# HIITMetagenomics/dsm-framework

Measured on AMD Instinct MI355X. Metric: enumerated substrings/sec (Emax=2.0), higher is better.
Workload: dtype u32

## Files before the change

### dsm-framework_amd/csrc/engine.hip

```cpp
#include <sched.h>

#include <algorithm>
#include <atomic>
#include <chrono>
#include <cmath>
#include <condition_variable>
#include <cstdlib>
#include <cstring>
#include <deque>
#include <map>
#include <functional>
#include <memory>
#include <mutex>
#include <sstream>
#include <thread>
#include <type_traits>

#include "common.h"
#include "scan.h"
#include "setorder.h"
#include "stream_parse.h"
#include "lfstep.h"
#include "entropy_tables.h"
#include "textemit.h"
// ... 833 lines not shown
        bitsv[i] = w < nw ? candbits[wc] : 0ull;
        basev[i] = wscan[wc];
    }
#pragma unroll
    for (int i = 0; i < NPT; ++i) {
        const u32 w = w0 + (u32)i * stride;
        const u64 bits = bitsv[i];
        if (!bits) continue;
        const u64 base = basev[i];
        const bool mine = (bits >> lane) & 1;
        const u32 v = w * 64 + lane;
        const u32 cnt = mine ? (a.d > 1 ? (u32)nT[v] : 1u) : 0u;
        const u32 k = (u32)(base & 0xFFFFFFFFu) + bits_below_lane(bits);
        u32 o = k;
        if (a.d > 1) o = (u32)(base >> 32) + (wave_inclusive_scan<u32>(cnt) - cnt);
        if (!mine) continue;
        cand_node[k] = v;
        cand_poff[k] = o;
        const u64 j = v;
        if (a.exact_order == 1) {
            const u64 ord = order[v];
            for (u32 q = 0; q < cnt; ++q) {
                u32 g = (u32)((ord >> (4 * q)) & 15);
                ids[o] = g; freqs[o] = (u64)x_freq<P>(x, g, j); ++o;
            }
        } else if (a.exact_order == 2) {
            const u16* ord = order16 + (size_t)v * a.d;
            for (u32 q = 0; q < cnt; ++q) {
                u32 g = ord[q];
                ids[o] = g; freqs[o] = (u64)x_freq<P>(x, g, j); ++o;
            }
        } else {
            for (u32 g = 0; g < a.d; ++g) {
                u64 f = (u64)x_freq<P>(x, g, j);
                if (f) { ids[o] = g; freqs[o] = f; ++o; }
            }
        }
    }
}

template <typename P>
__global__ void keep_kernel(u32 F, Xchg x, const uint2* __restrict__ sa, uint4* __restrict__ srec, u8* __restrict__ clen) {
    u32 v = blockIdx.x * blockDim.x + threadIdx.x;
    if (v >= F) return;
    const uint2 a = sa[v];
    const u64 f = (u64)x_freq<P>(x, 0, v);
    const u64 w = f | ((u64)(x_pl<P>(x, 0, v) >> 4) << 61);
    srec[v] = make_uint4(a.x, a.y, (u32)w, (u32)(w >> 32));
    clen[v] = (u8)((f < 128 ? 1u : 1u + (u32)((64 - __clzll((long long)f) + 7) >> 3)) + 2u);
}

template <typename T, typename OwnT>
__global__ __launch_bounds__(256) void up_kernel(u32 F, const OwnT* __restrict__ own, Kids kids, const T* __restrict__ child_agg,
                                                 T* __restrict__ agg) {
    const int lane = threadIdx.x & 63;
    const u32 nw = (F + 63) >> 6, stride = gridDim.x * 4;
    const u32 w0 = (u32)__builtin_amdgcn_readfirstlane((int)(xcd_block() * 4 + (threadIdx.x >> 6)));
    KidWave kw[NPT];
    T s[NPT];
#pragma unroll
    for (int i = 0; i < NPT; ++i) {
        const u32 w = w0 + (u32)i * stride, wc = w < nw ? w : 0u;
        const u32 v = wc * 64 + lane;
        s[i] = v < F ? (own ? (T)own[v] : (T)1) : (T)0;
        if (child_agg) kid_wave(kids, wc, kw[i]);
    }
    if (child_agg) {
        T g[NPT][4];
#pragma unroll
        for (int i = 0; i < NPT; ++i)
#pragma unroll
            for (int c = 0; c < 4; ++c) g[i][c] = child_agg[((kw[i].p[c] >> lane) & 1) ? kw[i].c[c] + bits_below_lane(kw[i].p[c]) : 0u];
#pragma unroll
        for (int i = 0; i < NPT; ++i)
#pragma unroll
            for (int c = 0; c < 4; ++c) s[i] += ((kw[i].p[c] >> lane) & 1) ? g[i][c] : (T)0;
    }
#pragma unroll
    for (int i = 0; i < NPT; ++i) {
        const u32 w = w0 + (u32)i * stride, v = w * 64 + lane;
        if (w < nw && v < F) agg[v] = s[i];
    }
}
template <typename T>
__global__ __launch_bounds__(256) void up_bits_kernel(u32 F, const u64* __restrict__ ownbits, Kids kids, const T* __restrict__ child_agg,
                                                      T* __restrict__ agg) {
    const int lane = threadIdx.x & 63;
    const u32 nw = (F + 63) >> 6, stride = gridDim.x * 4;
    const u32 w0 = (u32)__builtin_amdgcn_readfirstlane((int)(xcd_block() * 4 + (threadIdx.x >> 6)));
    KidWave kw[NPT];
    T s[NPT];
#pragma unroll
    for (int i = 0; i < NPT; ++i) {
        const u32 w = w0 + (u32)i * stride, wc = w < nw ? w : 0u;
        s[i] = ownbits ? (T)((ownbits[wc] >> lane) & 1) : (T)0;
        if (child_agg) kid_wave(kids, wc, kw[i]);
    }
    if (child_agg) {
        T g[NPT][4];
#pragma unroll
        for (int i = 0; i < NPT; ++i)
#pragma unroll
            for (int c = 0; c < 4; ++c) g[i][c] = child_agg[((kw[i].p[c] >> lane) & 1) ? kw[i].c[c] + bits_below_lane(kw[i].p[c]) : 0u];
#pragma unroll
        for (int i = 0; i < NPT; ++i)
#pragma unroll
            for (int c = 0; c < 4; ++c) s[i] += ((kw[i].p[c] >> lane) & 1) ? g[i][c] : (T)0;
    }
#pragma unroll
    for (int i = 0; i < NPT; ++i) {
        const u32 w = w0 + (u32)i * stride, v = w * 64 + lane;
        if (w < nw && v < F) agg[v] = s[i];
    }
}
template <typename T>
__global__ __launch_bounds__(256) void down_kernel(u32 F, const T* __restrict__ start, T lead, Kids kids,
                                                   const T* __restrict__ child_agg, T* __restrict__ child_start) {
    const int lane = threadIdx.x & 63;
    const u32 nw = (F + 63) >> 6, stride = gridDim.x * 4;
    const u32 w0 = (u32)__builtin_amdgcn_readfirstlane((int)(xcd_block() * 4 + (threadIdx.x >> 6)));
    KidWave kw[NPT];
    T s[NPT];
#pragma unroll
    for (int i = 0; i < NPT; ++i) {
        const u32 w = w0 + (u32)i * stride, wc = w < nw ? w : 0u;
        const u32 v = wc * 64 + lane;
        kid_wave(kids, wc, kw[i]);
        s[i] = start[v < F ? v : 0u] + lead;
    }
    T g[NPT][3];
#pragma unroll
    for (int i = 0; i < NPT; ++i)
#pragma unroll
        for (int c = 0; c < 3; ++c) {
            const bool need = ((kw[i].p[c] >> lane) & 1) && ((((kw[i].p[1] >> lane) & 1) << 1 | ((kw[i].p[2] >> lane) & 1) << 2 | ((kw[i].p[3] >> lane) & 1) << 3) >> (c + 1)) != 0;
            g[i][c] = child_agg[need ? kw[i].c[c] + bits_below_lane(kw[i].p[c]) : 0u];
        }
#pragma unroll
    for (int i = 0; i < NPT; ++i) {
        const u32 w = w0 + (u32)i * stride;
        if (w >= nw) continue;
        const u32 m = (u32)((kw[i].p[0] >> lane) & 1) | ((u32)((kw[i].p[1] >> lane) & 1) << 1) | ((u32)((kw[i].p[2] >> lane) & 1) << 2) |
                      ((u32)((kw[i].p[3] >> lane) & 1) << 3);
        T acc = s[i];
#pragma unroll
        for (int c = 0; c < 4; ++c) {
            if ((m >> c) & 1u) {
                child_start[kw[i].c[c] + bits_below_lane(kw[i].p[c])] = acc;
                if (c < 3 && (m >> (c + 1))) acc += g[i][c];
            }
        }
    }
}

struct RankSlot {
    u32 k, level;
    __device__ explicit operator u32() const { return level; }
};
__global__ void cand_rank_kernel(u32 ncand, const u32* __restrict__ cand_node, const u32* __restrict__ cand_poff, u32 npairs,
                                 const u32* __restrict__ start, const u32* __restrict__ sub, u32 level, RankSlot* __restrict__ slot,
                                 u32* __restrict__ npair, const uint4* __restrict__ crec) {
    u32 k = blockIdx.x * blockDim.x + threadIdx.x;
    if (k >= ncand) return;
    u32 v = crec ? crec[k].x : cand_node[k];
    u32 r = start[v] + sub[v] - 1;
    slot[r] = RankSlot{k, level};
    if (npair) npair[r] = crec ? 1u : (k + 1 < ncand ? cand_poff[k + 1] : npairs) - cand_poff[k];
}

struct LevelDev {
    const uint2* pw;
    const u32* cand_node;
    const u32* cand_poff;
    const uint4* crec;
    const u32* ids;
    const u64* freqs;
};

constexpr int EMIT_MAX_CHUNKS = 8;
struct ChunkBounds { u32 tb[EMIT_MAX_CHUNKS + 1]; int n; };
__global__ void chunk_bounds_kernel(ChunkBounds cbs, const u32* __restrict__ path_off, const u32* __restrict__ pair_off, u32* __restrict__ out) {
    const int c = threadIdx.x;
    if (c <= cbs.n) { out[2 * c] = path_off[cbs.tb[c]]; out[2 * c + 1] = pair_off ? pair_off[cbs.tb[c]] : cbs.tb[c]; }
}

constexpr u8 EV_DROP = 0, EV_KEEP = 1, EV_HOST = 2;
struct FillVerdict {
    u8* keep;
    double* ent;
    u32* rel_path;
    u32* rel_pair;
    u32* freq32;
    u32* counts;
    const double* terms;
    const double* logn;
    const u32* bounds;
    u32 chunk, d;
    double emin, emax;
};
__global__ __launch_bounds__(256) void tuple_fill_kernel(u32 nlev, const LevelDev* __restrict__ lv, const u32* __restrict__ path_off,
                                                         const u32* __restrict__ pair_off, const RankSlot* __restrict__ slot, char* __restrict__ paths,
                                                         u32* __restrict__ ids, u64* __restrict__ freqs, u32 rank_lo, u32 rank_hi, FillVerdict fv) {
    constexpr u32 LDS_LEVELS = 1024;
    __shared__ const uint2* s_pw[LDS_LEVELS];
    __shared__ u32 s_text[256];
    const u32 nl = nlev < LDS_LEVELS ? nlev : LDS_LEVELS;
    for (u32 q = threadIdx.x; q < nl; q += blockDim.x) s_pw[q] = lv[q].pw;
    {
        const u32 b = threadIdx.x;
        s_text[b] = ((0x54474341u >> (8 * (b & 3))) & 0xFFu) | (((0x54474341u >> (8 * ((b >> 2) & 3))) & 0xFFu) << 8) |
                    (((0x54474341u >> (8 * ((b >> 4) & 3))) & 0xFFu) << 16) | (((0x54474341u >> (8 * ((b >> 6) & 3))) & 0xFFu) << 24);
    }
    __syncthreads();
    const u32 r = rank_lo + blockIdx.x * blockDim.x + threadIdx.x;
    if (r >= rank_hi) return;
    const u32 p_first = path_off[r], p_end = path_off[r + 1];
    const u32 o_first = pair_off ? pair_off[r] : r, o_end = pair_off ? pair_off[r + 1] : r + 1;
    const u32 lvl = p_end - p_first;
    const u32 k = slot[r].k;
    const LevelDev L = lv[lvl];
    const bool one = L.crec != nullptr;
    const uint4 cr = one ? L.crec[k] : make_uint4(0u, 0u, 0u, 0u);
    const u32 b = one ? k : L.cand_poff[k];
    u64 sumN = fv.d;
    double sl = 0;
    bool beyond = false;
    for (u32 q = b, o = o_first; o < o_end; ++q, ++o) {
        const u64 fq = one ? (((u64)cr.w << 32) | cr.z) : L.freqs[q];
        if (ids) ids[o] = one ? 0u : L.ids[q];
        if (fv.freq32) fv.freq32[o] = (u32)fq; else freqs[o] = fq;
        sumN += fq;
        if (fv.keep && !beyond) {
            if (fq < TERM_TAB) sl += fv.terms[fq]; else beyond = true;
        }
    }
    if (fv.keep) {
        beyond = beyond || sumN >= LOGN_TAB;
        u8 verdict = EV_HOST;
        if (!beyond) {
            const double en = fv.logn[sumN] - sl / (double)sumN;
            if (fv.ent) fv.ent[r] = en;
            verdict = (fv.emax > 0 && (en < fv.emin || en > fv.emax)) ? EV_DROP : EV_KEEP;
        }
        const u32 pb0 = fv.bounds[2 * fv.chunk], qb0 = fv.bounds[2 * fv.chunk + 1];
        fv.keep[r] = verdict;
        fv.rel_path[r + fv.chunk] = p_first - pb0;
        if (fv.rel_pair) fv.rel_pair[r + fv.chunk] = o_first - qb0;
        if (r + 1 == rank_hi) {
// ... 151 lines not shown
    const u32 last = top_rank[v] + top_lf[v] - 1;
    const u64 val = rbase + cumk[last] + kop[last];
    rval[v] = val;
    atomicAdd(&chunk[last], 1u + varint_len(val));
}

constexpr u32 STREAM_LDS_LEVELS = 1024;
__global__ __launch_bounds__(256) void stream_chunk_kernel(u32 rank0, u32 nleaf, u32 nlev, const uint4* const* __restrict__ srec_tab, const u64* const* __restrict__ rval_tab,
                                                           const u64* __restrict__ leaf_id, const u64* __restrict__ chunk_off, const u32* __restrict__ kop,
                                                           u8* __restrict__ out) {
    __shared__ const uint4* s_rec[STREAM_LDS_LEVELS];
    const u32 nl = nlev < STREAM_LDS_LEVELS ? nlev : STREAM_LDS_LEVELS;
    for (u32 q = threadIdx.x; q < nl; q += blockDim.x) s_rec[q] = srec_tab[q];
    __syncthreads();
    const u32 r = rank0 + blockIdx.x * blockDim.x + threadIdx.x;
    if (r >= nleaf) return;
    const u64 id = leaf_id[r];
    u32 l = (u32)(id >> 32), v = (u32)id;
    const u32 ko = kop[r];
    u8* po = out + chunk_off[r] + 2ull * ko;
    u8* pc = po;
    bool inopen = true, inclose = true;
    while (l >= 1 && (inopen || inclose)) {
        const uint4 rec = (l < STREAM_LDS_LEVELS ? s_rec[l] : srec_tab[l])[v];
        if (inopen) {
            po -= 2;
            const unsigned short head = (unsigned short)('(' | ((0x54474341u >> (8 * (rec.y & 3u))) & 0xFFu) << 8);
            __builtin_memcpy(po, &head, 2);
            if (!(rec.y & SREC_FIRST)) inopen = false;
        }
        if (inclose) {
            const u64 fw = srec_word(rec);
            const u64 f = fw & SREC_FREQ_MASK;
            const u32 lc = (0x4E54474341300000ull >> (8 * ((u32)(fw >> 61) + 2))) & 0xFFu;
            if (l > 6 && f < (1ull << 32)) {
                u64 tok;
                u32 n;
                if (f < 128) { tok = f | 0x80; n = 1; }
                else { const u32 ln = (u32)((64 - __clzll((long long)f) + 7) >> 3); tok = (u64)ln | (f << 8); n = 1 + ln; }
                tok |= ((u64)lc | ((u64)')' << 8)) << (8 * n);
                n += 2;
                if (n & 4) { const u32 wv = (u32)tok; __builtin_memcpy(pc, &wv, 4); pc += 4; tok >>= 32; }
                if (n & 2) { const unsigned short wv = (unsigned short)tok; __builtin_memcpy(pc, &wv, 2); pc += 2; tok >>= 16; }
                if (n & 1) { *pc = (u8)tok; pc += 1; }
            } else {
                pc += put_varint(pc, f);
                if (l <= 6) { *pc++ = 'R'; pc += put_varint(pc, rval_tab[l][v]); }
                *pc++ = (u8)lc;
                *pc++ = ')';
            }
            if (!(rec.y & SREC_LAST)) inclose = false;
        }
        v = rec.x;
        --l;
    }
}

struct Arena {
    u8* base = nullptr;
    size_t cap = 0, off = 0;
    template <class T> T* get(size_t n) {
        size_t bytes = ((n ? n : 1) * sizeof(T) + 255) & ~(size_t)255;
        if (off + bytes > cap) return nullptr;
        T* p = reinterpret_cast<T*>(base + off);
        off += bytes;
        return p;
    }
};

struct LevelHost {
    u32 n = 0;
    u32* slot = nullptr;
    uint2* pw = nullptr;
    u64* kplane = nullptr;
    u32* kcum = nullptr;
    Kids kids() const { Kids k; k.plane = kplane; k.cum = kcum; return k; }
    u64* cand_bits = nullptr;
    u32 ncand = 0, npairs = 0;
    u32* cand_node = nullptr;
    u32* cand_poff = nullptr;
    uint4* crec = nullptr;
    u32* ids = nullptr;
    u64* freqs = nullptr;
    u32* sub = nullptr;
    uint4* srec = nullptr;
    u8* clen = nullptr;
    u32* lf = nullptr;
    u32* top_rank = nullptr;
    u32* top_lf = nullptr;
    u64* rval = nullptr;
};

static inline dim3 grid_for(u64 n, int t = 256) { return dim3((unsigned)((n + t - 1) / t)); }

#define ARENA_GET(var, T, n)                                                                        \
    do {                                                                                            \
        (var) = arena.get<T>(n);                                                                    \
        if (!(var)) return fail(DSM_E_CAPACITY, "device arena exhausted: use a longer prefix or a larger arena_bytes"); \
    } while (0)

static unsigned host_threads() {
    static unsigned n = 0;
    if (!n) {
        const char* e = getenv("DSM_HOST_THREADS");
        long v = e ? atol(e) : 0;
        if (v <= 0) {
            cpu_set_t cs;
            v = sched_getaffinity(0, sizeof cs, &cs) == 0 ? CPU_COUNT(&cs) : 1;
            if (v > 16) v = 16;
        }
        n = (unsigned)(v < 1 ? 1 : v);
    }
    return n;
}

struct RawBuf {
    void* p = nullptr;
    size_t cap = 0;
    void* ensure(size_t n) {
        if (n > cap) {
            free(p);
            cap = n + n / 4 + 4096;
            p = malloc(cap);
        }
        return p;
    }
    ~RawBuf() { free(p); }
};
struct PinBuf {
    void* p = nullptr;
    size_t cap = 0;
    int ensure(size_t n) {
        if (n <= cap) return 0;
        if (p) (void)hipHostFree(p);
        p = nullptr;
        cap = 0;
        size_t want = n + n / 4 + 4096;
        hipError_t e = hipHostMalloc(&p, want);
        if (e != hipSuccess) return fail(DSM_E_NOMEM, std::string("hipHostMalloc: ") + hipGetErrorString(e));
        cap = want;
        return 0;
    }
    ~PinBuf() { if (p) (void)hipHostFree(p); }
};
struct DevGrow {
    void* p = nullptr;
    size_t cap = 0;
    int ensure(size_t n) {
        if (n <= cap) return 0;
        if (p) (void)hipFree(p);
        p = nullptr;
        cap = 0;
        size_t want = n + n / 4 + 4096;
        hipError_t e = hipMalloc(&p, want);
        if (e != hipSuccess) return fail(DSM_E_NOMEM, std::string("hipMalloc: ") + hipGetErrorString(e));
        cap = want;
        return 0;
    }
    ~DevGrow() { if (p) (void)hipFree(p); }
};
struct EmitSet {
    DevGrow dev[11];
    bool one_pair = false, narrow = false;
    hipEvent_t ready = nullptr;
    static constexpr int MAX_CHUNKS = EMIT_MAX_CHUNKS;
    int nchunk = 1;
    u32 cb[MAX_CHUNKS + 1] = {0};
// ... 1248 lines not shown
            s.crec_cap = (u32)(room < (size_t)F ? room : (size_t)F);
        }
        const bool fold = s.crec_cap > 0;
        if (nbp > 1) {
            if (!merged) hipLaunchKernelGGL(lite_count_kernel, dim3((nbp + 63) / 64), dim3(256), 0, st, splane[0], (F + 63) >> 6, cntraw, nbp, 3u, fold ? 1u : 0u);
            exclusive_scan<u32, u32>(merged ? cnt4 : cntraw, cnt4, (size_t)(fold ? 5 : 4) * nbp, scan_tmp, d_totals, st);
        }
        const bool fused_filter = s.filtered && nbp > 1;
        if (fused_filter) {
            ao.fa = filter_args(F, depth, w.order_mode); ao.candbits = me.cand_bits; ao.wsum = cand_wsum;
            if (ao.single) ao.cand_copy = 1;
            else ao.filter_on = 1;
        }
        if (fold) { ao.crec = reinterpret_cast<uint4*>(carena.base + carena.off); ao.crec_cap = s.crec_cap; }
        if (nbp == 1) hipLaunchKernelGGL((advance_down_kernel<P>), dim3(1), dim3(256), 0, st, x, ao);
        else if (lean) hipLaunchKernelGGL((advance_single_kernel<P>), dim3((nbp + 3) / 4), dim3(256), 0, st, x, ao);
        else hipLaunchKernelGGL((advance_wave_kernel<P>), dim3(nbp), dim3(256), 0, st, x, ao);
        if (s.filtered) {
            if (int erc = emit_filter(me, F, depth, x, cur, w.order_mode, !fused_filter, fold)) return erc;
        }
        return 0;
    }

    int publish(Walk& w, Sweep& s) {
        const u32 F = w.F, nbp = (F + TILE - 1) / TILE;
        const int nxt = w.cur() ^ 1;
        PublishArgs pa;
        memset(&pa, 0, sizeof pa);
        pa.total = nbp == 1 ? d_pub_tot : d_totals;
        pa.cmax_base = s.x.base; pa.cmax_bpr = s.x.bpr; pa.cmax_world = (u32)world;
        if (s.filtered) pa.cand = d_totals64;
        if (s.crec_cap) {
            pa.total = cnt4 + (size_t)4 * nbp;
            pa.grand = d_totals;
            pa.cand = nullptr;
        }
        pa.clear = reinterpret_cast<u32*>(multi ? xsend : xrecv[nxt]);
        pa.packet = reinterpret_cast<uint4*>(h_totals + 304); pa.seq = ++pub_seq;
        pa.next = spec_mode ? d_dyn : nullptr;
        pa.bc_header = owner_mode ? reinterpret_cast<uint4*>(bc_buf) : nullptr;
        hipLaunchKernelGGL(publish_kernel, dim3(1), dim3(64), 0, st, pa);
        if (owner_mode) {
            const size_t bc_bytes = bcast_bytes(F);
            DSM_HIP(hipMemcpyAsync(bc_buf + 16, w.L[w.depth].kplane, bc_bytes - 16, hipMemcpyDeviceToDevice, st));
            w.owed.disarm();
            if (prm.bcast(prm.owner_ctx, owner, bc_buf, bc_bytes, (void*)st)) return fail(DSM_E_SINK, "bcast callback failed");
            stats.exchange_bytes_sent += bc_bytes * (u64)(world - 1);
        }
        if (spec_mode) { if (int rc = launch_lf(w, w.depth + 1, 0, w.w16, w.w9, s.slot, (u64)F * 4)) return rc; }
        u32 pk[4];
        if (int rc = wait_packet(pk)) return rc;
        s.Fn = decode_level(pk[1], &s.w16, &s.w9);
        s.spec_hit = spec_mode && s.Fn > 0 && s.Fn <= level_cap(s.w16) && s.w16 == w.w16 && s.w9 == w.w9;
        if (spec_mode && !s.spec_hit) --stats.expand_launches;
        h_totals[300] = pk[2]; h_totals[301] = pk[3];
        if (int rc = check_width(s.Fn, s.w16)) return rc;
        if (owner_mode) {
            if (!s.Fn) w.owed.arm(16);
            else w.owed.arm_next((size_t)level_bytes(s.Fn, s.w16, s.w9), xrecv[nxt], bcast_bytes(s.Fn));
        }
        return 0;
    }
    int wait_packet(u32 pk[4]) {
        volatile u32* fl = h_totals + 304;
        u32 spins = 0;
        while (*fl != pub_seq) {
            if ((++spins & 0xFFFFu) == 0 && hipStreamQuery(st) != hipErrorNotReady) {
                DSM_HIP(hipStreamSynchronize(st));
                if (*fl != pub_seq) return fail(DSM_E_HIP, "publish kernel did not report");
                break;
            }
            __builtin_ia32_pause();
        }
        std::atomic_thread_fence(std::memory_order_acquire);
        for (int q = 0; q < 4; ++q) pk[q] = fl[q];
        return 0;
    }

    int commit(Walk& w, const Sweep& s, LevelHost& child) {
        const u32 F = w.F, Fn = s.Fn;
        const int cur = w.cur(), nxt = cur ^ 1;
        arena.off = s.mark;
        child.n = Fn;
        if (!Fn) return 0;
        if (self_mode) child.slot = arena.get<u32>(Fn);
        if (!stream_mode) child.pw = arena.get<uint2>(Fn);
        if (int rc = alloc_kids(child)) return rc;
        if (s.spec_hit) {
            stats.expand_slots += Fn;
            stats.expand_column_bytes += (u64)Fn * col_bytes(s.w16, s.w9);
        } else {
            if (int rc = launch_lf(w, w.depth + 1, Fn, s.w16, s.w9, child.slot)) return rc;
        }
        const Kids kids = w.L[w.depth].kids();
        if (!(w.o.emit || w.o.capture)) {}
        else if (w.order_mode == 1)
            hipLaunchKernelGGL((order_kernel<P>), grid_for(F), dim3(256), 0, st, F, s.x, nT[cur], order[cur], kids, order[nxt]);
        else if (w.order_mode == 2 && d <= 64)
            hipLaunchKernelGGL((order_big_kernel<P, 64>), grid_for(F, 64), dim3(64), 0, st, F, s.x, nT[cur], order16[cur], kids, order16[nxt]);
        else if (w.order_mode == 2)
            hipLaunchKernelGGL((order_big_kernel<P, 273>), grid_for(F, 64), dim3(64), 0, st, F, s.x, nT[cur], order16[cur], kids, order16[nxt]);
        if (w.order_mode && w.o.seed && w.depth + 1 == w.o.seed->depth) {
            const std::vector<u16>& so = w.o.seed->ord[0];
            if (int rc = upload_order(nxt, so.data(), so.size())) return rc;
        }
        return 0;
    }

    int capture_level(Walk& w, u32 Fn, const u32* slot, const uint2* pw) {
        NodeOrder* cap = w.o.capture;
        if (!Fn || !cap || w.depth + 1 != cap->depth) return 0;
        const int nxt = w.cur() ^ 1;
        const bool client = owner_mode && !is_owner;
        std::vector<u32> hs(Fn);
        std::vector<u16> hn(Fn);
        if (slot) DSM_HIP(hipMemcpyAsync(hs.data(), slot, (size_t)Fn * sizeof(u32), hipMemcpyDeviceToHost, st));
        else if (stream_mode) {
            std::vector<uint2> hr(Fn);
            DSM_HIP(hipMemcpyAsync(hr.data(), sa[nxt], (size_t)Fn * sizeof(uint2), hipMemcpyDeviceToHost, st));
            DSM_HIP(hipStreamSynchronize(st));
            for (u32 v = 0; v < Fn; ++v) hs[v] = hr[v].y & 3u;
        } else {
            std::vector<uint2> hp(Fn);
            DSM_HIP(hipMemcpyAsync(hp.data(), pw, (size_t)Fn * sizeof(uint2), hipMemcpyDeviceToHost, st));
            DSM_HIP(hipStreamSynchronize(st));
            for (u32 v = 0; v < Fn; ++v) hs[v] = (hp[v].y >> (2 * (w.depth % PW_CHUNK))) & 3u;
        }
        if (!client) DSM_HIP(hipMemcpyAsync(hn.data(), nT[nxt], (size_t)Fn * sizeof(u16), hipMemcpyDeviceToHost, st));
        DSM_HIP(hipStreamSynchronize(st));
        const u32 order_mode = client ? 0u : w.order_mode;
        cap->sym.clear();
        cap->ord.clear();
        for (u32 v = 0; v < Fn; ++v) {
            cap->sym.push_back(hs[v] & 3);
            std::vector<u16> o(d == 1 || client ? 1 : hn[v]);
            if (order_mode == 1) {
                u64 ord = 0;
                DSM_HIP(hipMemcpy(&ord, order[nxt] + v, sizeof(u64), hipMemcpyDeviceToHost));
                for (u32 k = 0; k < hn[v]; ++k) o[k] = (u16)((ord >> (4 * k)) & 15);
            } else if (order_mode == 2) {
                DSM_HIP(hipMemcpy(o.data(), order16[nxt] + (size_t)v * d, (size_t)hn[v] * sizeof(u16), hipMemcpyDeviceToHost));
            }
            cap->ord.push_back(o);
        }
        return 0;
    }

    void count_level(const Walk& w) {
        if (w.trace) {
            if (owner_mode && !is_owner) fprintf(stderr, "dsm level prefix=%s depth=%u F=%u (client of rank %d)\n", w.prefix.c_str(), w.depth, w.F, owner);
            else fprintf(stderr, "dsm level prefix=%s depth=%u F=%u\n", w.prefix.c_str(), w.depth, w.F);
        }
        stats.union_nodes += w.depth >= 1 ? w.F : 0;
        if (w.F > stats.max_frontier) stats.max_frontier = w.F;
        ++stats.levels;
    }
    void step(Walk& w, u32 Fn, bool w16, bool w9) {
        w.F = Fn;
        ++w.depth;
        w.w16 = w16;
        w.w9 = w9;
    }

    int finish_prefix(Walk& w, dsm_tuple_sink tsink, dsm_byte_sink bsink, void* ctx) {
        const u32 nlev = (u32)w.L.size();
        if (stream_mode) {
// ... 50 lines not shown
            std::vector<u64> sh((size_t)COUNTER_SHARDS * 8);
            DSM_HIP(hipMemcpy(sh.data(), d_counters, sh.size() * sizeof(u64), hipMemcpyDeviceToHost));
            for (int k = 0; k < COUNTER_SHARDS; ++k)
                for (int c = 0; c < NCOUNTERS; ++c) hc[c] += sh[(size_t)k * 8 + c];
#ifdef DSM_CLOCK_PROBE
            if (sh[7]) {
                double dur = 0, ramp = 0, tail = 0, meanbusy = 0;
                int nl = 0;
                const double W = (double)lfgeo.blocks * lfgeo.waves_per_block;
                for (int k = 1; k + 2 < COUNTER_SHARDS; k += 3) {
                    const u64 s0 = ~sh[(size_t)k * 8 + 6], s9 = sh[(size_t)k * 8 + 7], e0 = ~sh[(size_t)(k + 1) * 8 + 6], e9 = sh[(size_t)(k + 1) * 8 + 7];
                    if (!s9 || e9 - s0 < 5000) continue;
                    const double ms = (double)sh[(size_t)(k + 2) * 8 + 6] / W, me = (double)sh[(size_t)(k + 2) * 8 + 7] / W;
                    dur += (double)(e9 - s0); ramp += (double)(s9 - s0); tail += (double)(e9 - e0); meanbusy += me - ms; ++nl;
                }
                fprintf(stderr, "clock probe: %.1f MHz; %d launches >= 50 us: duration %.2f ms, first-to-last wave start %.2f ms, first-to-last wave end %.2f ms, mean wave busy %.2f ms\n",
                        (double)sh[6] / (double)sh[7] * 100.0, nl, dur * 1e-5, ramp * 1e-5, tail * 1e-5, meanbusy * 1e-5);
            }
#endif
        }
        stats.reported += hc[0];
        stats.lf_steps += hc[1];
        stats.rank_ops += hc[2];
        stats.index_lines += hc[3];
        stats.record_bytes += hc[4];
        stats.records_read += hc[5];
        return 0;
    }

    FilterArgs filter_args(u32 F, u32 depth, u32 order_mode) const {
        FilterArgs fa;
        fa.F = F; fa.depth = depth; fa.d = d; fa.pmin = prm.pmin; fa.pmax = prm.pmax; fa.mindepth = prm.mindepth;
        fa.emin = prm.emin; fa.emax = prm.emax; fa.exact_order = order_mode;
        return fa;
    }
    int emit_alloc(LevelHost& me, u32 F) {
        EARENA_GET(me.cand_bits, u64, ((size_t)F + 63) / 64);
        return 0;
    }
    int emit_filter(LevelHost& me, u32 F, u32 depth, const Xchg& xp, int cur, u32 order_mode, bool run_kernel, bool stored = false) {
        const FilterArgs fa = filter_args(F, depth, order_mode);
        if (run_kernel)
            hipLaunchKernelGGL((filter_kernel<P>), grid_npt(F), dim3(256), 0, st, fa, xp, nT[cur], me.kids(), samechild, me.cand_bits, cand_wsum);
        if (!stored) exclusive_scan<u64, u64>(cand_wsum, cand_wscan, ((size_t)F + 63) / 64, scan_tmp64, d_totals64, st);
        return 0;
    }
    int emit_store(LevelHost& me, u32 F, u32 depth, const Xchg& xp, int cur, u32 order_mode, u32 stored_cap = 0) {
        const FilterArgs fa = filter_args(F, depth, order_mode);
        u64 tot = 0;
        memcpy(&tot, h_totals + 300, sizeof tot);
        me.ncand = (u32)(tot & 0xFFFFFFFFu);
        me.npairs = (u32)(tot >> 32);
        if (stored_cap && me.ncand <= stored_cap) {
            if (me.ncand) {
                me.crec = carena.get<uint4>(me.ncand);
                if (!me.crec) return fail(DSM_E_HIP, "candidate arena: the block that held the records cannot be claimed");
            }
            stats.candidates += me.ncand;
            return 0;
        }
        if (stored_cap)
            exclusive_scan<u64, u64>(cand_wsum, cand_wscan, ((size_t)F + 63) / 64, scan_tmp64, d_totals64, st);
        if (me.ncand) {
            u32 nc = me.ncand;
            me.ncand = 0;
            EARENA_GET(me.cand_node, u32, nc);
            EARENA_GET(me.cand_poff, u32, nc);
            EARENA_GET(me.ids, u32, me.npairs);
            EARENA_GET(me.freqs, u64, me.npairs);
            me.ncand = nc;
            hipLaunchKernelGGL((cand_store_kernel<P>), grid_npt(F), dim3(256), 0, st, fa, xp, nT[cur], order[cur], order16[cur], me.cand_bits, cand_wscan,
                               me.cand_node, me.cand_poff, me.ids, me.freqs);
        }
        stats.candidates += me.ncand;
        return 0;
    }

    int finish_mine(std::vector<LevelHost>& L, u32 nlev, dsm_tuple_sink sink, void* ctx, bool* ready) {
        u64 ncand_total = 0;
        for (u32 l = 1; l < nlev; ++l) ncand_total += L[l].ncand;
        if (ncand_total == 0) return 0;
        if (ncand_total > 0xFFFFFFF0ull) return fail(DSM_E_CAPACITY, "more than 2^32 candidate tuples in one prefix: use a longer prefix");
        const u32 nt = (u32)ncand_total;
        for (u32 l = nlev; l-- > 1;) {
            EARENA_GET(L[l].sub, u32, L[l].n);
            const u32* child_sub = l + 1 < nlev ? L[l + 1].sub : nullptr;
            hipLaunchKernelGGL((up_bits_kernel<u32>), grid_npt(L[l].n), dim3(256), 0, st, L[l].n, L[l].cand_bits, L[l].kids(), child_sub, L[l].sub);
        }
        const bool text_mode = text_sink_ != nullptr;
        const bool one_pair = d == 1 && !text_mode;
        const bool narrow = one_pair && sizeof(P) == 4 && !trie_mode;
        u32* npair = nullptr;
        if (!one_pair) EARENA_GET(npair, u32, nt);
        u32 maxn = 1;
        for (u32 l = 0; l < nlev; ++l) maxn = L[l].n > maxn ? L[l].n : maxn;
        u32* startbuf[2];
        EARENA_GET(startbuf[0], u32, maxn);
        EARENA_GET(startbuf[1], u32, maxn);
        RankSlot* slot;
        EARENA_GET(slot, RankSlot, nt);
        DSM_HIP(hipMemsetAsync(startbuf[0], 0, sizeof(u32), st));
        for (u32 l = 0; l + 1 < nlev; ++l) {
            u32* s_cur = startbuf[l & 1];
            u32* s_next = startbuf[(l + 1) & 1];
            hipLaunchKernelGGL((down_kernel<u32>), grid_npt(L[l].n), dim3(256), 0, st, L[l].n, s_cur, 0u, L[l].kids(), L[l + 1].sub, s_next);
            if (L[l + 1].ncand)
                hipLaunchKernelGGL(cand_rank_kernel, grid_for(L[l + 1].ncand), dim3(256), 0, st, L[l + 1].ncand, L[l + 1].cand_node, L[l + 1].cand_poff,
                                   L[l + 1].npairs, s_next, L[l + 1].sub, l + 1, slot, npair, L[l + 1].crec);
        }
        std::vector<LevelDev> lv(nlev);
        u64 path_bytes = 0, npairs = 0;
        for (u32 l = 0; l < nlev; ++l) {
            lv[l].pw = L[l].pw; lv[l].cand_node = L[l].cand_node; lv[l].cand_poff = L[l].cand_poff; lv[l].crec = L[l].crec;
            lv[l].ids = L[l].ids; lv[l].freqs = L[l].freqs;
            if (l && L[l].ncand) { path_bytes += (u64)l * L[l].ncand; npairs += L[l].crec ? L[l].ncand : L[l].npairs; }
        }
        if (path_bytes > 0xFFFFFFFFull || npairs > 0xFFFFFFFFull) return fail(DSM_E_CAPACITY, "more than 2^32 path bytes or pairs in one prefix: use a longer prefix");
        LevelDev* d_lv;
        EARENA_GET(d_lv, LevelDev, nlev);
        DSM_HIP(hipMemcpyAsync(d_lv, lv.data(), nlev * sizeof(LevelDev), hipMemcpyHostToDevice, st));
        EmitSet& E = emitter.acquire();
        E.device = device;
        if (!E.ready) DSM_HIP(hipEventCreateWithFlags(&E.ready, hipEventDisableTiming));
        if (!copy_stream) DSM_HIP(hipStreamCreateWithFlags(&copy_stream, hipStreamNonBlocking));
        if (int rc = E.dev[0].ensure(((size_t)nt + 1) * 4)) return rc;
        if (!one_pair) { if (int rc = E.dev[1].ensure(((size_t)nt + 1) * 4)) return rc; }
        u32* path_off = (u32*)E.dev[0].p;
        u32* pair_off = one_pair ? nullptr : (u32*)E.dev[1].p;
        u32* stmp;
        EARENA_GET(stmp, u32, scan_tmp_elems(nt) + 8);
        exclusive_scan<RankSlot, u32>(slot, path_off, nt, stmp, d_totals, st);
        if (!one_pair) exclusive_scan<u32, u32>(npair, pair_off, nt, stmp, d_totals + 1, st);
        DSM_HIP(hipMemcpyAsync(path_off + nt, d_totals, sizeof(u32), hipMemcpyDeviceToDevice, st));
        if (!one_pair) DSM_HIP(hipMemcpyAsync(pair_off + nt, d_totals + 1, sizeof(u32), hipMemcpyDeviceToDevice, st));
        static const u64 chunk_unit = [] {
            const char* e = getenv("DSM_EMIT_CHUNK_TUPLES");
            const long long n = e ? atoll(e) : 0;
            return n > 0 ? (u64)n : (u64)(1u << 20);
        }();
        ChunkBounds cbs;
        cbs.n = nt >= 4 * chunk_unit ? 4 : (nt >= 2 * chunk_unit ? 2 : 1);
        for (int c = 0; c <= cbs.n; ++c) cbs.tb[c] = (u32)((u64)nt * c / cbs.n);
        u32* d_bounds;
        EARENA_GET(d_bounds, u32, 2 * (EmitSet::MAX_CHUNKS + 1));
        hipLaunchKernelGGL(chunk_bounds_kernel, dim3(1), dim3(64), 0, st, cbs, path_off, pair_off, d_bounds);
        DSM_HIP(hipMemcpyAsync(h_bounds, d_bounds, 2 * (cbs.n + 1) * sizeof(u32), hipMemcpyDeviceToHost, st));
        if (!bounds_landed) DSM_HIP(hipEventCreateWithFlags(&bounds_landed, hipEventDisableTiming));
        DSM_HIP(hipEventRecord(bounds_landed, st));
        const bool no_ids = d == 1;
        if (!no_ids) { if (int rc = E.dev[2].ensure((size_t)npairs * 4)) return rc; }
        if (!narrow) { if (int rc = E.dev[3].ensure((size_t)npairs * 8)) return rc; }
        if (int rc = E.dev[4].ensure((size_t)path_bytes)) return rc;
        u32* d_ids = no_ids ? nullptr : (u32*)E.dev[2].p;
        u64* d_freqs = narrow ? nullptr : (u64*)E.dev[3].p;
        char* d_paths = (char*)E.dev[4].p;
        emitter.text_sink = text_sink_;
        FillVerdict fv;
        memset(&fv, 0, sizeof fv);
        if (!text_mode) {
            const size_t nrel = (size_t)nt + EmitSet::MAX_CHUNKS + 1;
            if (int rc = E.pin[0].ensure(nrel * 4)) return rc;
            if (!one_pair) { if (int rc = E.pin[1].ensure(nrel * 4)) return rc; }
            if (!no_ids) { if (int rc = E.pin[2].ensure((size_t)npairs * 4)) return rc; }
            if (int rc = E.pin[3].ensure((size_t)npairs * 8)) return rc;
            if (int rc = E.pin[4].ensure((size_t)path_bytes)) return rc;
            if (int rc = E.pin[5].ensure((size_t)nt * 8)) return rc;
            if (int rc = E.pin[6].ensure((size_t)nt)) return rc;
            if (int rc = E.pin[9].ensure(2 * EmitSet::MAX_CHUNKS * sizeof(u32))) return rc;
            if (!one_pair) { if (int rc = E.dev[5].ensure((size_t)nt * 8)) return rc; }
            if (int rc = E.dev[6].ensure((size_t)nt)) return rc;
            if (int rc = E.dev[7].ensure(nrel * 4)) return rc;
            if (!one_pair) { if (int rc = E.dev[8].ensure(nrel * 4)) return rc; }
            if (narrow) {
                if (int rc = E.pin[10].ensure((size_t)nt * 4)) return rc;
                if (int rc = E.dev[10].ensure((size_t)nt * 4)) return rc;
            }
            if (int rc = E.dev[9].ensure(2 * EmitSet::MAX_CHUNKS * sizeof(u32))) return rc;
            if (!d_terms) {
                if (int rc = dalloc(d_terms, (size_t)TERM_TAB)) return rc;
                if (int rc = dalloc(d_logn, (size_t)LOGN_TAB)) return rc;
                DSM_HIP(hipMemcpyAsync(d_terms, term_table(), (size_t)TERM_TAB * 8, hipMemcpyHostToDevice, st));
                DSM_HIP(hipMemcpyAsync(d_logn, logn_table(), (size_t)LOGN_TAB * 8, hipMemcpyHostToDevice, st));
            }
            DSM_HIP(hipMemsetAsync(E.dev[9].p, 0, 2 * EmitSet::MAX_CHUNKS * sizeof(u32), st));
            fv.keep = (u8*)E.dev[6].p; fv.rel_path = (u32*)E.dev[7].p;
            if (!one_pair) { fv.ent = (double*)E.dev[5].p; fv.rel_pair = (u32*)E.dev[8].p; }
            if (narrow) fv.freq32 = (u32*)E.dev[10].p;
            fv.terms = d_terms; fv.logn = d_logn; fv.d = d; fv.emin = prm.emin; fv.emax = prm.emax; fv.bounds = d_bounds;
        }
        E.nchunk = cbs.n;
        E.one_pair = one_pair; E.narrow = narrow;
// ... 431 lines not shown
```

Measured before the change: 3.734 billion.

## Tile up/down sweeps via LDS staging and store subtree counts in u16

Replaces the per-wave scattered child gathers and scatters in the up and down rank sweeps with a tiled scheme. Each wave handles four consecutive words, loads the contiguous child run for each of the four planes into LDS in coalesced form, computes from LDS, and writes child starts back coalesced. Deep levels whose subtree counts provably fit in 16 bits get u16 sub arrays, decided from the w9 flag and fmin, which halves their traffic. The cost is 16KB of LDS per block, a fixed run capacity of 256 children per plane per tile, and more kernel template variants.

```diff
diff --git a/dsm-framework_amd/csrc/engine.hip b/dsm-framework_amd/csrc/engine.hip
--- a/dsm-framework_amd/csrc/engine.hip
+++ b/dsm-framework_amd/csrc/engine.hip
@@ -939,88 +939,160 @@
         if (w < nw && v < F) agg[v] = s[i];
     }
 }
-template <typename T>
-__global__ __launch_bounds__(256) void up_bits_kernel(u32 F, const u64* __restrict__ ownbits, Kids kids, const T* __restrict__ child_agg,
+struct TileKids {
+    u64 p[4][4];
+    u32 base[4];
+    u32 n[4];
+};
+__device__ __forceinline__ void tile_kids(const Kids& k, u32 w0, u32 nw, TileKids& t) {
+#pragma unroll
+    for (int c = 0; c < 4; ++c) { t.base[c] = k.cum[(size_t)w0 * 4 + c]; t.n[c] = 0; }
+#pragma unroll
+    for (int q = 0; q < 4; ++q) {
+        const bool in = w0 + q < nw;
+#pragma unroll
+        for (int c = 0; c < 4; ++c) {
+            const u64 pl = k.plane[(size_t)(w0 + q) * 4 + c];
+            t.p[q][c] = in ? pl : 0ull;
+            t.n[c] += (u32)__popcll(t.p[q][c]);
+        }
+    }
+}
+template <int NC, typename CT>
+__device__ __forceinline__ void tile_runs_in(const TileKids& t, const CT* __restrict__ child, u32* run, int lane) {
+    CT g[NC][4];
+#pragma unroll
+    for (int c = 0; c < NC; ++c)
+#pragma unroll
+        for (int j = 0; j < 4; ++j) {
+            g[c][j] = (CT)0;
+            if ((u32)j * 64 < t.n[c]) {
+                const u32 e = (u32)j * 64 + (u32)lane;
+                g[c][j] = child[t.base[c] + (e < t.n[c] ? e : t.n[c] - 1)];
+            }
+        }
+#pragma unroll
+    for (int c = 0; c < NC; ++c)
+#pragma unroll
+        for (int j = 0; j < 4; ++j)
+            if ((u32)j * 64 < t.n[c]) run[c * 256 + j * 64 + lane] = (u32)g[c][j];
+}
+__device__ __forceinline__ void wave_lds_fence() {
+    __builtin_amdgcn_fence(__ATOMIC_RELEASE, "wavefront");
+    __builtin_amdgcn_wave_barrier();
+    __builtin_amdgcn_fence(__ATOMIC_ACQUIRE, "wavefront");
+}
+template <typename CT, typename T>
+__global__ __launch_bounds__(256) void up_tile_kernel(u32 F, const u64* __restrict__ ownbits, Kids kids, const CT* __restrict__ child_agg,
                                                       T* __restrict__ agg) {
+    __shared__ u32 stage[4][4 * 256];
     const int lane = threadIdx.x & 63;
-    const u32 nw = (F + 63) >> 6, stride = gridDim.x * 4;
-    const u32 w0 = (u32)__builtin_amdgcn_readfirstlane((int)(xcd_block() * 4 + (threadIdx.x >> 6)));
-    KidWave kw[NPT];
-    T s[NPT];
-#pragma unroll
-    for (int i = 0; i < NPT; ++i) {
-        const u32 w = w0 + (u32)i * stride, wc = w < nw ? w : 0u;
-        s[i] = ownbits ? (T)((ownbits[wc] >> lane) & 1) : (T)0;
-        if (child_agg) kid_wave(kids, wc, kw[i]);
-    }
+    const u32 wi = (u32)__builtin_amdgcn_readfirstlane((int)(threadIdx.x >> 6));
+    const u32 nw = (F + 63) >> 6;
+    const u32 w0 = (u32)__builtin_amdgcn_readfirstlane((int)((xcd_block() * 4 + wi) * 4));
+    if (w0 >= nw) return;
+    u32* run = stage[wi];
+    u64 own[4] = {0, 0, 0, 0};
+    if (ownbits) {
+#pragma unroll
+        for (int q = 0; q < 4; ++q) own[q] = ownbits[w0 + q < nw ? w0 + q : w0];
+    }
+    u32 s[4];
+#pragma unroll
+    for (int q = 0; q < 4; ++q) s[q] = (u32)((own[q] >> lane) & 1);
     if (child_agg) {
-        T g[NPT][4];
-#pragma unroll
-        for (int i = 0; i < NPT; ++i)
-#pragma unroll
-            for (int c = 0; c < 4; ++c) g[i][c] = child_agg[((kw[i].p[c] >> lane) & 1) ? kw[i].c[c] + bits_below_lane(kw[i].p[c]) : 0u];
-#pragma unroll
-        for (int i = 0; i < NPT; ++i)
-#pragma unroll
-            for (int c = 0; c < 4; ++c) s[i] += ((kw[i].p[c] >> lane) & 1) ? g[i][c] : (T)0;
-    }
-#pragma unroll
-    for (int i = 0; i < NPT; ++i) {
-        const u32 w = w0 + (u32)i * stride, v = w * 64 + lane;
-        if (w < nw && v < F) agg[v] = s[i];
-    }
-}
-template <typename T>
-__global__ __launch_bounds__(256) void down_kernel(u32 F, const T* __restrict__ start, T lead, Kids kids,
-                                                   const T* __restrict__ child_agg, T* __restrict__ child_start) {
+        TileKids t;
+        tile_kids(kids, w0, nw, t);
+        tile_runs_in<4, CT>(t, child_agg, run, lane);
+        wave_lds_fence();
+        u32 pre[4] = {0, 0, 0, 0};
+#pragma unroll
+        for (int q = 0; q < 4; ++q)
+#pragma unroll
+            for (int c = 0; c < 4; ++c) {
+                const u32 x = run[c * 256 + pre[c] + bits_below_lane(t.p[q][c])];
+                s[q] += ((t.p[q][c] >> lane) & 1) ? x : 0u;
+                pre[c] += (u32)__popcll(t.p[q][c]);
+            }
+    }
+#pragma unroll
+    for (int q = 0; q < 4; ++q) {
+        const u32 v = (w0 + q) * 64 + lane;
+        if (w0 + q < nw && v < F) agg[v] = (T)s[q];
+    }
+}
+template <typename CT>
+__global__ __launch_bounds__(256) void down_tile_kernel(u32 F, const u32* __restrict__ start, Kids kids, const CT* __restrict__ child_agg,
+                                                        u32* __restrict__ child_start) {
+    __shared__ u32 stage[4][4 * 256];
     const int lane = threadIdx.x & 63;
-    const u32 nw = (F + 63) >> 6, stride = gridDim.x * 4;
-    const u32 w0 = (u32)__builtin_amdgcn_readfirstlane((int)(xcd_block() * 4 + (threadIdx.x >> 6)));
-    KidWave kw[NPT];
-    T s[NPT];
-#pragma unroll
-    for (int i = 0; i < NPT; ++i) {
-        const u32 w = w0 + (u32)i * stride, wc = w < nw ? w : 0u;
-        const u32 v = wc * 64 + lane;
-        kid_wave(kids, wc, kw[i]);
-        s[i] = start[v < F ? v : 0u] + lead;
-    }
-    T g[NPT][3];
-#pragma unroll
-    for (int i = 0; i < NPT; ++i)
+    const u32 wi = (u32)__builtin_amdgcn_readfirstlane((int)(threadIdx.x >> 6));
+    const u32 nw = (F + 63) >> 6;
+    const u32 w0 = (u32)__builtin_amdgcn_readfirstlane((int)((xcd_block() * 4 + wi) * 4));
+    if (w0 >= nw) return;
+    u32* run = stage[wi];
+    u32 s[4];
+#pragma unroll
+    for (int q = 0; q < 4; ++q) {
+        const u32 v = (w0 + q) * 64 + lane;
+        s[q] = start[w0 + q < nw && v < F ? v : 0u];
+    }
+    TileKids t;
+    tile_kids(kids, w0, nw, t);
+    tile_runs_in<3, CT>(t, child_agg, run, lane);
+    wave_lds_fence();
+    u32 g[4][3], pre[4] = {0, 0, 0, 0};
+#pragma unroll
+    for (int q = 0; q < 4; ++q)
 #pragma unroll
         for (int c = 0; c < 3; ++c) {
-            const bool need = ((kw[i].p[c] >> lane) & 1) && ((((kw[i].p[1] >> lane) & 1) << 1 | ((kw[i].p[2] >> lane) & 1) << 2 | ((kw[i].p[3] >> lane) & 1) << 3) >> (c + 1)) != 0;
-            g[i][c] = child_agg[need ? kw[i].c[c] + bits_below_lane(kw[i].p[c]) : 0u];
-        }
-#pragma unroll
-    for (int i = 0; i < NPT; ++i) {
-        const u32 w = w0 + (u32)i * stride;
-        if (w >= nw) continue;
-        const u32 m = (u32)((kw[i].p[0] >> lane) & 1) | ((u32)((kw[i].p[1] >> lane) & 1) << 1) | ((u32)((kw[i].p[2] >> lane) & 1) << 2) |
-                      ((u32)((kw[i].p[3] >> lane) & 1) << 3);
-        T acc = s[i];
+            g[q][c] = run[c * 256 + pre[c] + bits_below_lane(t.p[q][c])];
+            pre[c] += (u32)__popcll(t.p[q][c]);
+        }
+#pragma unroll
+    for (int c = 0; c < 4; ++c) pre[c] = 0;
+#pragma unroll
+    for (int q = 0; q < 4; ++q) {
+        u32 acc = s[q];
 #pragma unroll
         for (int c = 0; c < 4; ++c) {
-            if ((m >> c) & 1u) {
-                child_start[kw[i].c[c] + bits_below_lane(kw[i].p[c])] = acc;
-                if (c < 3 && (m >> (c + 1))) acc += g[i][c];
-            }
-        }
-    }
+            if ((t.p[q][c] >> lane) & 1) {
+                run[c * 256 + pre[c] + bits_below_lane(t.p[q][c])] = acc;
+                if (c < 3) acc += g[q][c];
+            }
+            pre[c] += (u32)__popcll(t.p[q][c]);
+        }
+    }
+    wave_lds_fence();
+    u32 o[4][4];
+#pragma unroll
+    for (int c = 0; c < 4; ++c)
+#pragma unroll
+        for (int j = 0; j < 4; ++j) {
+            o[c][j] = 0;
+            if ((u32)j * 64 < t.n[c]) o[c][j] = run[c * 256 + j * 64 + lane];
+        }
+#pragma unroll
+    for (int c = 0; c < 4; ++c)
+#pragma unroll
+        for (int j = 0; j < 4; ++j) {
+            const u32 e = (u32)j * 64 + (u32)lane;
+            if ((u32)j * 64 < t.n[c] && e < t.n[c]) child_start[t.base[c] + e] = o[c][j];
+        }
 }
 
 struct RankSlot {
     u32 k, level;
     __device__ explicit operator u32() const { return level; }
 };
+template <typename ST>
 __global__ void cand_rank_kernel(u32 ncand, const u32* __restrict__ cand_node, const u32* __restrict__ cand_poff, u32 npairs,
-                                 const u32* __restrict__ start, const u32* __restrict__ sub, u32 level, RankSlot* __restrict__ slot,
+                                 const u32* __restrict__ start, const ST* __restrict__ sub, u32 level, RankSlot* __restrict__ slot,
                                  u32* __restrict__ npair, const uint4* __restrict__ crec) {
     u32 k = blockIdx.x * blockDim.x + threadIdx.x;
     if (k >= ncand) return;
     u32 v = crec ? crec[k].x : cand_node[k];
-    u32 r = start[v] + sub[v] - 1;
+    u32 r = start[v] + (u32)sub[v] - 1;
     slot[r] = RankSlot{k, level};
     if (npair) npair[r] = crec ? 1u : (k + 1 < ncand ? cand_poff[k + 1] : npairs) - cand_poff[k];
 }
@@ -1338,7 +1410,9 @@
     uint4* crec = nullptr;
     u32* ids = nullptr;
     u64* freqs = nullptr;
-    u32* sub = nullptr;
+    bool w9 = false;
+    void* sub = nullptr;
+    bool sub16 = false;
     uint4* srec = nullptr;
     u8* clen = nullptr;
     u32* lf = nullptr;
@@ -2753,6 +2827,7 @@
         const int cur = w.cur(), nxt = cur ^ 1;
         arena.off = s.mark;
         child.n = Fn;
+        child.w9 = s.w9;
         if (!Fn) return 0;
         if (self_mode) child.slot = arena.get<u32>(Fn);
         if (!stream_mode) child.pw = arena.get<uint2>(Fn);
@@ -2969,10 +3044,31 @@
         if (ncand_total == 0) return 0;
         if (ncand_total > 0xFFFFFFF0ull) return fail(DSM_E_CAPACITY, "more than 2^32 candidate tuples in one prefix: use a longer prefix");
         const u32 nt = (u32)ncand_total;
+        static const u32 sub16_max = [] {
+            const char* e = getenv("DSM_RANK_SUB16_MAX");
+            const long long n = e ? atoll(e) : 65535;
+            return (u32)(n < 0 ? 0 : (n > 65535 ? 65535 : n));
+        }();
+        u32 first16 = nlev;
+        if (!trie_mode && sub16_max) {
+            const u64 per_depth = (u64)d * (511u / (prm.fmin > 1u ? prm.fmin : 1u));
+            for (u32 l = nlev; l-- > 1;) {
+                if (!L[l].w9 || (u64)(nlev - l) * per_depth > sub16_max) break;
+                first16 = l;
+            }
+        }
         for (u32 l = nlev; l-- > 1;) {
-            EARENA_GET(L[l].sub, u32, L[l].n);
-            const u32* child_sub = l + 1 < nlev ? L[l + 1].sub : nullptr;
-            hipLaunchKernelGGL((up_bits_kernel<u32>), grid_npt(L[l].n), dim3(256), 0, st, L[l].n, L[l].cand_bits, L[l].kids(), child_sub, L[l].sub);
+            LevelHost& me = L[l];
+            me.sub16 = l >= first16;
+            if (me.sub16) { u16* p; EARENA_GET(p, u16, me.n); me.sub = p; }
+            else { u32* p; EARENA_GET(p, u32, me.n); me.sub = p; }
+            const void* child_sub = l + 1 < nlev ? L[l + 1].sub : nullptr;
+            if (me.sub16)
+                hipLaunchKernelGGL((up_tile_kernel<u16, u16>), grid_npt(me.n), dim3(256), 0, st, me.n, me.cand_bits, me.kids(), (const u16*)child_sub, (u16*)me.sub);
+            else if (l + 1 < nlev && L[l + 1].sub16)
+                hipLaunchKernelGGL((up_tile_kernel<u16, u32>), grid_npt(me.n), dim3(256), 0, st, me.n, me.cand_bits, me.kids(), (const u16*)child_sub, (u32*)me.sub);
+            else
+                hipLaunchKernelGGL((up_tile_kernel<u32, u32>), grid_npt(me.n), dim3(256), 0, st, me.n, me.cand_bits, me.kids(), (const u32*)child_sub, (u32*)me.sub);
         }
         const bool text_mode = text_sink_ != nullptr;
         const bool one_pair = d == 1 && !text_mode;
@@ -2990,10 +3086,15 @@
         for (u32 l = 0; l + 1 < nlev; ++l) {
             u32* s_cur = startbuf[l & 1];
             u32* s_next = startbuf[(l + 1) & 1];
-            hipLaunchKernelGGL((down_kernel<u32>), grid_npt(L[l].n), dim3(256), 0, st, L[l].n, s_cur, 0u, L[l].kids(), L[l + 1].sub, s_next);
-            if (L[l + 1].ncand)
-                hipLaunchKernelGGL(cand_rank_kernel, grid_for(L[l + 1].ncand), dim3(256), 0, st, L[l + 1].ncand, L[l + 1].cand_node, L[l + 1].cand_poff,
-                                   L[l + 1].npairs, s_next, L[l + 1].sub, l + 1, slot, npair, L[l + 1].crec);
+            const LevelHost& ch = L[l + 1];
+            if (ch.sub16) hipLaunchKernelGGL((down_tile_kernel<u16>), grid_npt(L[l].n), dim3(256), 0, st, L[l].n, s_cur, L[l].kids(), (const u16*)ch.sub, s_next);
+            else hipLaunchKernelGGL((down_tile_kernel<u32>), grid_npt(L[l].n), dim3(256), 0, st, L[l].n, s_cur, L[l].kids(), (const u32*)ch.sub, s_next);
+            if (ch.ncand && ch.sub16)
+                hipLaunchKernelGGL((cand_rank_kernel<u16>), grid_for(ch.ncand), dim3(256), 0, st, ch.ncand, ch.cand_node, ch.cand_poff, ch.npairs, s_next,
+                                   (const u16*)ch.sub, l + 1, slot, npair, ch.crec);
+            else if (ch.ncand)
+                hipLaunchKernelGGL((cand_rank_kernel<u32>), grid_for(ch.ncand), dim3(256), 0, st, ch.ncand, ch.cand_node, ch.cand_poff, ch.npairs, s_next,
+                                   (const u32*)ch.sub, l + 1, slot, npair, ch.crec);
         }
         std::vector<LevelDev> lv(nlev);
         u64 path_bytes = 0, npairs = 0;
```

After: 3.713 billion. No clear change (-0.6%).
